# facebookresearch/holo_diffusion

Hardware: AMD Instinct MI355X
Metric: denoise-steps/sec + rendered-rays/sec, 64^3x32 grid @400^2 render (higher is better)
Workload: dtype f32

## Files before the change

### holo_diffusion_amd/csrc/holo_kernels.h

```cpp
#pragma once
#include <stddef.h>
#include <stdint.h>
#include <string.h>

#include "../../include/holo_abi.h"
#include "attn_plan.h"
#include "bwd_plan.h"
#include "conv_plan.h"
#include "conv_weights.h"
#include "holo_knobs.h"
#include "render_plan.h"

struct HoloCtx {
  int device;
  int num_cus;
  int deterministic = 0;
};

namespace holo {

int conv_launch(const ConvParams& p, void* stream);
int conv_s2_bf16_launch(const ConvParams& p, void* stream);
int conv1x1_qkv_bf16_launch(const ConvParams& p, void* stream);
int conv1x1_bf16_stream_launch(const ConvParams& p, void* stream);
int conv_wino3_launch(const ConvParams& p, void* stream);
int conv_bf16p_launch(const ConvParams& p, void* stream);
int repack_conv_weight_wino3_launch(const float* w, float* out, int Cout, int Cin, int src_taps, int CoutP, int CinP,
                                    void* stream);

int gemm_launch(const GemmParams& p, void* stream);
inline int gemm_batch_launch(const float* A, int lda, const float* B, int ldb, int b_kmajor, float* C, int ldc, int M, int N,
                             int K, int nb, int64_t sa, int64_t sb, int64_t sc, void* stream) {
  GemmParams g;
  memset(&g, 0, sizeof g);
  g.A = A, g.B = B, g.C = C;
  g.M = M, g.Nn = N, g.K = K;
  g.lda = lda, g.ldb = ldb, g.ldc = ldc;
  g.nb0 = nb, g.nb1 = 1;
  g.sa0 = sa, g.sb0 = sb, g.sc0 = sc;
  g.b_kmajor = b_kmajor;
  g.alpha = 1.f;
  return gemm_launch(g, stream);
}

int flash_attn_launch(const AttnParams& p, void* stream);
int flash_attn_bf16v2_launch(const AttnParams& p, void* work, int out_bf16, int ksplit, int lazy, void* stream, int packed = 0);

int softmax_rows_launch(float* s, int64_t rows, int cols, void* stream);

int ncdhw_to_ndhwc_launch(const float* in, float* out, int N, int C, int64_t V, int tanh_flag, void* stream,
                          int out_bf16 = 0);
int ndhwc_to_ncdhw_launch(const float* in, float* out, int N, int C, int64_t V, void* stream, int in_bf16 = 0);
int f32_to_bf16_launch(const float* in, float* out_bf16, int64_t n, void* stream);

int gn_stats_launch(const float* x, double* partial, int N, int C, int64_t V, void* stream, int x_bf16 = 0);

int gn_finalize_launch(const double* part0, int C0, int B0, const double* part1, int C1, int B1, int N, int64_t V,
                       int groups, float eps, const float* gamma, const float* beta, const float* film,
                       int film_stride, int film_cout, float* coef, void* stream, float* moments = nullptr);

int time_embed_launch(const int64_t* t, int N, int mc, int ted, const float* w1, const float* b1, const float* w2,
                      const float* b2, float* emb, float* emb_silu, int load_kind, void* stream);

int rows_linear_launch(const float* in, const float* w, const float* bias, float* out, int N, int rows, int K,
                       void* stream);

int ddpm_step_launch(const float* tables, int T, const int64_t* timesteps, int batch, int64_t per, const float* x_t,
                     const float* model_out, const float* noise, int clip, float* sample, float* pred_xstart,
                     void* stream);
int ddpm_step_philox_launch(const float* tables, int T, const int64_t* timesteps, int batch, int64_t per, const float* x_t,
                            const float* model_out, uint64_t seed, const uint32_t* row_streams, uint64_t offset, int clip,
                            float* sample, float* pred_xstart, float* noise_out, int ncdhw_channels, void* stream);
int ddim_step_launch(const float* coefs, int batch, int64_t per, const float* x_t, const float* model_out,
                     const float* noise, int clip, float* sample, float* pred_xstart, void* stream);
int ddim_step_philox_launch(const float* coefs, int batch, int64_t per, const float* x_t, const float* model_out,
                            uint64_t seed, const uint32_t* row_streams, uint64_t offset, int clip, float* sample,
                            float* pred_xstart, float* noise_out, int ncdhw_channels, void* stream);
int ddpm_step_guided_launch(const float* tables, int T, const int64_t* timesteps, const float* variances, int batch,
                            int64_t per, const float* x_t, const float* model_out, const float* grad, const float* noise,
                            int clip, float* sample, float* pred_xstart, void* stream);
int ddpm_step_guided_philox_launch(const float* tables, int T, const int64_t* timesteps, const float* variances, int batch,
                                   int64_t per, const float* x_t, const float* model_out, const float* grad, uint64_t seed,
                                   const uint32_t* row_streams, uint64_t offset, int clip, float* sample,
                                   float* pred_xstart, float* noise_out, int ncdhw_channels, void* stream);
int ddim_step_guided_launch(const float* coefs, int batch, int64_t per, const float* x_t, const float* model_out,
                            const float* grad, const float* noise, int clip, float* sample, float* pred_xstart,
                            void* stream);
int ddim_step_guided_philox_launch(const float* coefs, int batch, int64_t per, const float* x_t, const float* model_out,
                                   const float* grad, uint64_t seed, const uint32_t* row_streams, uint64_t offset, int clip,
                                   float* sample, float* pred_xstart, float* noise_out, int ncdhw_channels, void* stream);
int dpm_step_launch(const float* coefs, int batch, int64_t per, const float* x_t, const float* model_out,
                    const float* hist1, const float* hist2, int clip, float* sample, float* pred_xstart, void* stream);
int ddpm_step_inpaint_launch(const float* tables, int T, const int64_t* timesteps, const float* known_coefs, int batch,
                             int64_t per, int channels, int ncdhw, const float* x_t, const float* model_out,
                             const float* x0_known, const float* mask, const float* noise, const float* noise_known,
                             int clip, float* sample, float* pred_xstart, void* stream);
int ddpm_step_inpaint_philox_launch(const float* tables, int T, const int64_t* timesteps, const float* known_coefs, int batch,
                                    int64_t per, int channels, int ncdhw, const float* x_t, const float* model_out,
                                    const float* x0_known, const float* mask, uint64_t seed, const uint32_t* row_streams,
                                    uint64_t offset, int clip, float* sample, float* pred_xstart, float* noise_out,
                                    float* noise_known_out, void* stream);
int q_sample_launch(const float* coefs, int batch, int64_t per, const float* x, const float* noise, float* out, void* stream);
int q_sample_philox_launch(const float* coefs, int batch, int64_t per, const float* x, uint64_t seed,
                           const uint32_t* row_streams, uint64_t offset, float* out, float* noise_out, int ncdhw_channels,
                           void* stream);
int tanh_launch(const float* x, float* y, int64_t n, void* stream);
int copy_sys_launch(const float* src, float* dst, int64_t n, void* stream);
#define HIP_TRY(expr)                                                                        \
  do {                                                                                       \
    hipError_t _e = (expr);                                                                  \
    if (_e != hipSuccess) {                                                                  \
      holo::set_error("%s failed: %s (%s:%d)", #expr, hipGetErrorString(_e), __FILE__, __LINE__); \
// ... 307 lines not shown
```

### holo_diffusion_amd/csrc/holo_knobs.h

```cpp
#pragma once

#include <stdint.h>
#include <stdlib.h>

namespace holo {

#ifdef HOLO_EMU
constexpr bool EMU_BUILD = true;
#else
constexpr bool EMU_BUILD = false;
#endif

constexpr int64_t KNOB_UNSET = INT64_MIN;

#define HOLO_KNOBS(X)                                                                                                      \
  X(num_cus, "HOLO_NUM_CUS", POS, 0, CTX, "planners size grids and split-K for this many CUs (default: the device's)")     \
  X(conv_wino, "HOLO_CONV_WINO", INT, 1, HANDLE, "0: no Winograd copies of the conv weights (forward and dgrad)")          \
  X(conv_wino3, "HOLO_CONV_WINO3", INT, 1, HANDLE_PLAN, "0: no F(2x2x2, 3x3x3) copies / conv_wino3_kernel never chosen")   \
  X(keep_intermediates, "HOLO_KEEP_INTERMEDIATES", CH, '1', HANDLE,                                                        \
    "1: the plan releases no activation, holo_unet_fetch_block works")                                                     \
  X(render_v1, "HOLO_RENDER_V1", SET, 0, HANDLE, "the ray-per-column render kernel for everything")                        \
  X(render2_nw, "HOLO_RENDER2_NW", INT, 0, HANDLE, "8: the 8-wave form of render2_kernel's 12-wave configurations")        \
  X(render2_nrm_nw, "HOLO_RENDER2_NRM_NW", INT, 0, HANDLE,                                                                 \
    "8: rendered normals two waves per SIMD instead of 10 waves (the emulation build always runs 8)")                      \
  X(render_wgs, "HOLO_RENDER_WGS", POS, 0, HANDLE, "persistent render workgroups (default: one per CU)")                   \
  X(render_xcd, "HOLO_RENDER_XCD", RAW, KNOB_UNSET, HANDLE,                                                                \
    "XCD ranges of the render tile order (default 8; 2 in the emulation build; <= 1: plain order)")                        \
  X(render_tail, "HOLO_RENDER_TAIL", RAW, KNOB_UNSET, HANDLE,                                                              \
    "4-ray tiles at the end of every XCD range handed out as single rays (default: about two rounds; 3 in the "            \
    "emulation build; 0: off)")                                                                                            \
  X(render_static_tiles, "HOLO_RENDER_STATIC_TILES", SET, 0, HANDLE, "static tile stride instead of the dynamic hand-out") \
  X(render_timeline, "HOLO_RENDER_TIMELINE", SET, 0, HANDLE, "per-phase clocks of every render launch (synchronises!)")    \
  X(mlp_mean_bwd_chunk, "HOLO_MLP_MEAN_BWD_CHUNK", POS, 0, HANDLE,                                                         \
    "voxels per chunk of holo_mlp_mean_backward (default: what fits 4 GiB of rows; the emulation build: always 2048)")     \
  X(conv_wino_small, "HOLO_CONV_WINO_SMALL", INT, 1, PLAN, "0: under-filled levels take 64-voxel tiles, not Winograd")     \
  X(conv_force_tz2, "HOLO_CONV_FORCE_TZ2", INT, 0, PLAN, "1: 128-voxel tiles (hence the Winograd kernels) on small grids") \
  X(conv_qkv_fused, "HOLO_CONV_QKV_FUSED", INT, 1, PLAN, "0: row-tile qkv convolution + attn_pack_kernel")                 \
  X(conv1x1_bf16_stream, "HOLO_CONV1X1_BF16_STREAM", INT, 1, PLAN, "0: the row-tile kernel for bf16 1x1x1 convolutions")   \
  X(conv1x1_stream_min_m, "HOLO_CONV1X1_STREAM_MIN_M", INT, 131072, PLAN,                                                  \
    "rows from which a raw-input fp32 1x1x1 convolution streams (0: never)")                                               \
  X(conv1x1_small, "HOLO_CONV1X1_SMALL", INT, 1, PLAN, "0: the row-tile kernel for the fp32 attention's 1x1x1 convs")      \
  X(conv_s2t, "HOLO_CONV_S2T", INT, -1, PLAN, "stride-2 bf16 halo kernel: 0 never, 1 wherever defined (default: by fill)") \
  X(conv_bf16t, "HOLO_CONV_BF16T", INT, -1, PLAN, "bf16 wide-tile kernel: 0 never, 1 everywhere (default: by fill / K)")   \
  X(conv_bf16p, "HOLO_CONV_BF16P", INT, -1, PLAN,                                                                          \
    "its persistent form: 0 never, 1 every wide-tile launch, 2 activated input too (default: raw input)")                  \
  X(conv_bf16p_wgs, "HOLO_CONV_BF16P_WGS", INT, 0, PLAN, "at most this many persistent workgroups (0: no cap)")            \
  X(conv_wino3_min_items, "HOLO_CONV_WINO3_MIN_ITEMS", INT, KNOB_UNSET, PLAN,                                              \
    "work items from which conv_wino3_kernel runs (default: num_cus / 2)")                                                 \
  X(conv_wino3_up, "HOLO_CONV_WINO3_UP", INT, 1, PLAN,                                                                     \
    "0: upsampling convolutions on conv_wino3_kernel's generic form (64 pseudo-taps), not its 27-tap form")               \
  X(no_skip_fusion, "HOLO_NO_SKIP_FUSION", SET, 0, PLAN, "a ResBlock's 1x1x1 skip always as its own launch")               \
  X(skip_fusion_below_r, "HOLO_SKIP_FUSION_BELOW_R", RAW, 64, PLAN,                                                        \
    "exact fp32: the skip is fused into the second convolution below this grid edge")                                      \
  X(side_lane_cus, "HOLO_SIDE_LANE_CUS", INT, 128, PLAN,                                                                   \
    "exact fp32 inference: CUs the skip half of a split up-path concat convolution is planned for (0: nothing is split)")  \
  X(side_lane_min_r, "HOLO_SIDE_LANE_MIN_R", INT, 32, PLAN, "smallest grid edge whose concat convolutions are split")      \
  X(side_lane_fork_r, "HOLO_SIDE_LANE_FORK_R", INT, 8, PLAN,                                                               \
    "the side lane starts in front of the first descent level whose grid edge is at most this")                            \
  X(no_flash_attn, "HOLO_NO_FLASH_ATTN", SET, 0, PLAN, "attention as GEMM + softmax + GEMM")                               \
  X(bf16_flash_min_t, "HOLO_BF16_FLASH_MIN_T", RAW, 1024, PLAN, "tokens from which the bf16 mode takes its bf16 attention") \
  X(flash_split, "HOLO_FLASH_SPLIT", INT, 0, PLAN, "key splits of the fp32 attention, clamped to [1, T/128] (0: by fill)") \
  X(flash_v2_ksplit, "HOLO_FLASH_V2_KSPLIT", INT, 0, PLAN,                                                                 \
    "key splits of the bf16 attention: 1..8 dividing T into multiples of 128, else ignored")                               \
  X(attn_exact, "HOLO_ATTN_EXACT", SET, 0, PLAN, "bf16 attention: the exact loop alone, no LAZY pass")                     \
  X(debug_timestep_load, "HOLO_DEBUG_TIMESTEP_LOAD", INT, 0, PLAN, "how time_embed_kernel loads the timesteps (see it)")   \
  X(dgrad_s2_direct, "HOLO_DGRAD_S2_DIRECT", CH, '1', PLAN, "1: conv_dgrad_s2_kernel for every Downsample dgrad")          \
  X(wgrad_tiles, "HOLO_WGRAD_TILES", POS, 0, PLAN, "> 0: the tile weight-gradient kernel instead of the row-staged one")   \
  X(wgrad_reduce_tile_min, "HOLO_WGRAD_REDUCE_TILE_MIN", RAW, 1024, PLAN,                                                  \
    "64-element tiles from which the weight-gradient reduce runs its tile form")                                           \
  X(debug_plan, "HOLO_DEBUG_PLAN", SET, 0, PLAN, "[plan] lines on stderr: what every convolution / attention launches")    \
  X(viewpool_bwd_v1, "HOLO_VIEWPOOL_BWD_V1", CH, '1', CALL, "1: the register-accumulating view-pool backward kernel")      \
  HOLO_KNOBS_DEV(X)

#ifdef HOLO_DEV_PROBES
#define HOLO_KNOBS_DEV(X)                                                                                                  \
  X(viewpool_bwd_probe, "HOLO_VIEWPOOL_BWD_PROBE", RAW, KNOB_UNSET, CALL,                                                  \
    "view-pool backward: 0 no pass 2, 2 pass 2 without its atomics, 10 + k the atomics of map k alone")                    \
  X(viewpool_bwd_occ, "HOLO_VIEWPOOL_BWD_OCC", CH, '3', CALL, "view-pool backward: 3 = the 166-register build")
#else
#define HOLO_KNOBS_DEV(X)
#endif

typedef int64_t knob_INT_t, knob_RAW_t, knob_POS_t;
typedef bool knob_SET_t, knob_CH_t;
static inline int64_t knob_INT(const char* e, int64_t dflt) { return e && e[0] ? strtoll(e, nullptr, 10) : dflt; }
static inline int64_t knob_RAW(const char* e, int64_t dflt) { return e ? atoll(e) : dflt; }
static inline bool knob_SET(const char* e, int) { return e != nullptr; }
static inline bool knob_CH(const char* e, char c) { return e && e[0] == c; }
static inline int64_t knob_POS(const char* e, int) { return e && atoll(e) > 0 ? atoll(e) : 0; }

struct Knobs {
#define HOLO_KNOB_FIELD(field, env, kind, dflt, when, doc) knob_##kind##_t field;
  HOLO_KNOBS(HOLO_KNOB_FIELD)
#undef HOLO_KNOB_FIELD
  static Knobs from_env() {
    Knobs k;
#define HOLO_KNOB_READ(field, env, kind, dflt, when, doc) k.field = knob_##kind(getenv(env), dflt);
    HOLO_KNOBS(HOLO_KNOB_READ)
#undef HOLO_KNOB_READ
    return k;
  }
};

}
```

### holo_diffusion_amd/csrc/kernels_misc.hip

```cpp
#include <stdlib.h>

#include "holo_common.h"
#include "holo_kernels.h"

namespace holo {
namespace {

__global__ __launch_bounds__(256) void ncdhw_to_ndhwc_kernel(const float* __restrict__ in, float* __restrict__ out,
                                                             int C, int64_t V, int tanh_flag, int out_bf16) {
  __shared__ float tile[32][33];
  const int n = blockIdx.z;
  const int64_t v0 = (int64_t)blockIdx.x * 32;
  const int c0 = blockIdx.y * 32;
  const int tx = threadIdx.x & 31, ty = threadIdx.x >> 5;
  in += (int64_t)n * C * V;
  const int64_t obase = (int64_t)n * C * V;
  for (int j = ty; j < 32; j += 8) {
    const int c = c0 + j;
    const int64_t v = v0 + tx;
    float x = 0.f;
    if (c < C && v < V) x = in[(int64_t)c * V + v];
    if (tanh_flag) x = tanhf(x);
    tile[j][tx] = x;
  }
  __syncthreads();
  for (int j = ty; j < 32; j += 8) {
    const int64_t v = v0 + j;
    const int c = c0 + tx;
    if (c < C && v < V) {
      if (out_bf16)
        reinterpret_cast<uint16_t*>(out)[obase + v * C + c] = (uint16_t)(pack_bf16x2(tile[tx][j], 0.f) & 0xffffu);
      else
        out[obase + v * C + c] = tile[tx][j];
    }
  }
}

__global__ __launch_bounds__(256) void f32_to_bf16_kernel(const float4* __restrict__ in, float4* __restrict__ out, int64_t n8) {
  for (int64_t i = (int64_t)blockIdx.x * blockDim.x + threadIdx.x; i < n8; i += (int64_t)gridDim.x * blockDim.x) {
    const float4 a = in[2 * i], b = in[2 * i + 1];
    out[i] = make_float4(__uint_as_float(pack_bf16x2(a.x, a.y)), __uint_as_float(pack_bf16x2(a.z, a.w)),
                         __uint_as_float(pack_bf16x2(b.x, b.y)), __uint_as_float(pack_bf16x2(b.z, b.w)));
  }
}

__global__ __launch_bounds__(256) void ndhwc_to_ncdhw_kernel(const float* __restrict__ in, float* __restrict__ out,
                                                             int C, int64_t V, int in_bf16) {
  __shared__ float tile[32][33];
  const int n = blockIdx.z;
  const int64_t v0 = (int64_t)blockIdx.x * 32;
  const int c0 = blockIdx.y * 32;
  const int tx = threadIdx.x & 31, ty = threadIdx.x >> 5;
  const int64_t ibase = (int64_t)n * C * V;
  out += (int64_t)n * C * V;
  for (int j = ty; j < 32; j += 8) {
    const int64_t v = v0 + j;
// ... 45 lines not shown
      fs[3] += t.w;
      fq[0] += t.x * t.x;
      fq[1] += t.y * t.y;
      fq[2] += t.z * t.z;
      fq[3] += t.w * t.w;
      if (++cnt == 32) {
#pragma unroll
        for (int e = 0; e < 4; ++e) {
          ds[e] += fs[e];
          dq[e] += fq[e];
          fs[e] = 0.f;
          fq[e] = 0.f;
        }
        cnt = 0;
      }
    }
#pragma unroll
    for (int e = 0; e < 4; ++e) {
      ds[e] += fs[e];
      dq[e] += fq[e];
    }
  }
#pragma unroll
  for (int e = 0; e < 4; ++e) {
    red[tid * 8 + e] = ds[e];
    red[tid * 8 + 4 + e] = dq[e];
  }
  __syncthreads();
  if (tid < cq) {
    double s[8] = {0, 0, 0, 0, 0, 0, 0, 0};
    for (int r = 0; r < rows; ++r)
#pragma unroll
      for (int e = 0; e < 8; ++e) s[e] += red[(r * cq + tid) * 8 + e];
    double* dst = partial + (((int64_t)n * gridDim.x + blockIdx.x) * C + tid * 4) * 2;
#pragma unroll
    for (int e = 0; e < 4; ++e) {
      dst[e * 2 + 0] = s[e];
      dst[e * 2 + 1] = s[4 + e];
    }
  }
}

__device__ __forceinline__ double shfl_xor_f64(double v, int mask) {
  unsigned long long b;
  memcpy(&b, &v, 8);
  const float lo = __shfl_xor(__uint_as_float((uint32_t)(b & 0xffffffffull)), mask);
  const float hi = __shfl_xor(__uint_as_float((uint32_t)(b >> 32)), mask);
  b = (unsigned long long)__float_as_uint(lo) | ((unsigned long long)__float_as_uint(hi) << 32);
  double r;
  memcpy(&r, &b, 8);
  return r;
}

__global__ __launch_bounds__(256) void gn_finalize_kernel(const double* __restrict__ part0, int C0, int B0,
                                                          const double* __restrict__ part1, int C1, int B1, int64_t V,
                                                          int groups, float eps, const float* __restrict__ gamma,
                                                          const float* __restrict__ beta,
                                                          const float* __restrict__ film, int film_stride,
                                                          int film_cout, float* __restrict__ coef,
                                                          float* __restrict__ moments) {
  __shared__ double rs[4], rq[4];
  const int g = blockIdx.x, n = blockIdx.y, tid = threadIdx.x;
  const int Cin = C0 + C1;
  const int cpg = Cin / groups;
  float pg = 0.f, pb = 0.f, psc = 0.f, psh = 0.f;
  if (tid < cpg) {
    const int c = g * cpg + tid;
    pg = gamma[c];
    pb = beta[c];
    if (film) {
      psc = film[(int64_t)n * film_stride + c];
      psh = film[(int64_t)n * film_stride + film_cout + c];
    }
  }
  double s = 0.0, sq = 0.0;
  {
    const int c_lo = g * cpg, c_hi = c_lo + cpg;
    const int c_mid = c_lo < C0 ? (c_hi < C0 ? c_hi : C0) : c_lo;
    for (int half = 0; half < 2; ++half) {
      const int ca = half == 0 ? c_lo : c_mid, cb = half == 0 ? c_mid : c_hi;
      const int nch = cb - ca;
      if (nch <= 0) continue;
      const double* p = half == 0 && ca < C0 ? part0 : part1;
      const int Cs = p == part0 ? C0 : C1, B = p == part0 ? B0 : B1;
      const int cs0 = p == part0 ? ca : ca - C0;
      const int64_t total = (int64_t)B * nch;
      const double* base = p + ((int64_t)n * B * Cs + cs0) * 2;
      const bool pow2 = (nch & (nch - 1)) == 0;
      const int sh = 31 - __builtin_clz((unsigned)nch);
      auto rec = [&](int64_t j64) -> int64_t {
        const unsigned j = (unsigned)j64;
        const unsigned q = pow2 ? (j >> sh) : j / (unsigned)nch;
        const unsigned r = pow2 ? (j & (unsigned)(nch - 1)) : j - q * (unsigned)nch;
        return ((int64_t)q * Cs + r) * 2;
      };
      int64_t i = tid;
      for (; i + 15 * 256 < total; i += 16 * 256) {
        double2 v[16];
#pragma unroll
        for (int u = 0; u < 16; ++u) {
          const int64_t j = i + u * 256;
          v[u] = *reinterpret_cast<const double2*>(base + rec(j));
        }
#pragma unroll
        for (int u = 0; u < 16; ++u) {
          s += v[u].x;
          sq += v[u].y;
        }
      }
      for (; i + 7 * 256 < total; i += 8 * 256) {
        double2 v[8];
#pragma unroll
        for (int u = 0; u < 8; ++u) {
          const int64_t j = i + u * 256;
          v[u] = *reinterpret_cast<const double2*>(base + rec(j));
        }
#pragma unroll
        for (int u = 0; u < 8; ++u) {
          s += v[u].x;
          sq += v[u].y;
        }
      }
      for (; i < total; i += 256) {
        const double2 v = *reinterpret_cast<const double2*>(base + rec(i));
        s += v.x;
        sq += v.y;
      }
    }
  }
#pragma unroll
  for (int o = 32; o >= 1; o >>= 1) {
    s += shfl_xor_f64(s, o);
    sq += shfl_xor_f64(sq, o);
  }
  if ((tid & 63) == 0) {
    rs[tid >> 6] = s;
    rq[tid >> 6] = sq;
  }
  __syncthreads();
  if (tid < cpg) {
    const int c = g * cpg + tid;
    const double cnt = (double)cpg * (double)V;
    const double mean = (((rs[0] + rs[1]) + rs[2]) + rs[3]) / cnt;
    double var = (((rq[0] + rq[1]) + rq[2]) + rq[3]) / cnt - mean * mean;
    if (var < 0.0) var = 0.0;
    const double rstd = 1.0 / sqrt(var + (double)eps);
    double a = rstd * (double)pg;
    double b = (double)pb - mean * a;
    if (film) {
      const double sc = 1.0 + (double)psc;
      const double sh = (double)psh;
      a *= sc;
      b = b * sc + sh;
    }
    coef[((int64_t)n * Cin + c) * 2 + 0] = (float)a;
    coef[((int64_t)n * Cin + c) * 2 + 1] = (float)b;
    if (moments) {
      moments[((int64_t)n * Cin + c) * 2 + 0] = (float)mean;
      moments[((int64_t)n * Cin + c) * 2 + 1] = (float)rstd;
    }
  }
}

__global__ __launch_bounds__(256) void time_embed_kernel(const int64_t* __restrict__ t, int mc, int ted,
                                                         const float* __restrict__ w1, const float* __restrict__ b1,
                                                         const float* __restrict__ w2, const float* __restrict__ b2,
                                                         float* __restrict__ emb, float* __restrict__ emb_silu,
                                                         int load_kind) {
  __shared__ float te[256];
  __shared__ float h1[1024];
  const int n = blockIdx.x;
  const int tid = threadIdx.x;
  float tv;
  if (load_kind == 1) {
    tv = (float)t[n];
  } else if (load_kind == 2) {
    const int64_t* tp = t + n;
    HOLO_LAUNDER(tp);
    tv = (float)*tp;
  } else {
    tv = (float)holo_ld_sys(t + n);
  }
  const int half = mc / 2;
  for (int i = tid; i < mc; i += 256) {
    float v = 0.f;
    if (i < 2 * half) {
      const int k = i < half ? i : i - half;
      const float freq = expf((-9.210340371976184f * (float)k) / (float)half);
      const float arg = tv * freq;
      v = i < half ? cosf(arg) : sinf(arg);
    }
    te[i] = v;
  }
  __syncthreads();
  for (int j = tid; j < ted; j += 256) {
    float acc = 0.f;
    const float* w = w1 + (int64_t)j * mc;
    for (int k = 0; k < mc; ++k) acc = fmaf(w[k], te[k], acc);
    acc += b1[j];
    h1[j] = acc / (1.0f + expf(-acc));
  }
  __syncthreads();
  for (int j = tid; j < ted; j += 256) {
    float acc = 0.f;
    const float* w = w2 + (int64_t)j * ted;
    for (int k = 0; k < ted; ++k) acc = fmaf(w[k], h1[k], acc);
    acc += b2[j];
    emb[(int64_t)n * ted + j] = acc;
    emb_silu[(int64_t)n * ted + j] = acc / (1.0f + expf(-acc));
  }
}

__global__ __launch_bounds__(256) void rows_linear_kernel(const float* __restrict__ in, const float* __restrict__ w,
                                                          const float* __restrict__ bias, float* __restrict__ out,
// ... 568 lines not shown
    const int ci = cc * 32 + (lane >> 4) * 8 + e2 * 2;
    const float v0 = (ci < Cin && co < Cout) ? holo_ld_sys(w + ((int64_t)co * Cin + ci) * taps + tap) : 0.f;
    const float v1 = (ci + 1 < Cin && co < Cout) ? holo_ld_sys(w + ((int64_t)co * Cin + ci + 1) * taps + tap) : 0.f;
    const uint32_t h = pack_bf16x2(v0, v1);
    const float r0 = v0 - __uint_as_float(h << 16), r1 = v1 - __uint_as_float(h & 0xffff0000u);
    const uint32_t m = pack_bf16x2(r0, r1);
    const uint32_t l = pack_bf16x2(r0 - __uint_as_float(m << 16), r1 - __uint_as_float(m & 0xffff0000u));
    o32[i] = h;
    o32[total + i] = m;
    o32[2 * total + i] = l;
    {
      const int nc16 = CinP >> 4, ns32 = CoutP >> 5;
      int64_t b2 = i >> 8;
      const int sl2 = (int)(b2 % ns32);
      b2 /= ns32;
      const int cc2 = (int)(b2 % nc16);
      const int tap2 = (int)(b2 / nc16);
      const int co2 = sl2 * 32 + (lane & 31);
      const int ci2 = cc2 * 16 + (lane >> 5) * 8 + e2 * 2;
      const float u0 = (ci2 < Cin && co2 < Cout) ? w[((int64_t)co2 * Cin + ci2) * taps + tap2] : 0.f;
      const float u1 = (ci2 + 1 < Cin && co2 < Cout) ? w[((int64_t)co2 * Cin + ci2 + 1) * taps + tap2] : 0.f;
      o32[3 * total + i] = pack_bf16x2(u0, u1);
    }
  }
}

}

int ncdhw_to_ndhwc_launch(const float* in, float* out, int N, int C, int64_t V, int tanh_flag, void* stream, int out_bf16) {
  dim3 grid((unsigned)cdiv(V, 32), (unsigned)cdiv(C, 32), (unsigned)N);
  HOLO_LAUNCH(ncdhw_to_ndhwc_kernel, grid, dim3(256), stream, in, out, C, V, tanh_flag, out_bf16);
  return 0;
}
int ndhwc_to_ncdhw_launch(const float* in, float* out, int N, int C, int64_t V, void* stream, int in_bf16) {
  dim3 grid((unsigned)cdiv(V, 32), (unsigned)cdiv(C, 32), (unsigned)N);
  HOLO_LAUNCH(ndhwc_to_ncdhw_kernel, grid, dim3(256), stream, in, out, C, V, in_bf16);
  return 0;
}

int gn_stats_launch(const float* x, double* partial, int N, int C, int64_t V, void* stream, int x_bf16) {
  if ((C & 3) || (C >> 2) > 256) {
    set_error("gn_stats: unsupported C=%d", C);
    return -1;
  }
  int B, vpb;
  gn_stats_geometry(C, V, &B, &vpb);
  dim3 grid((unsigned)B, (unsigned)N);
  HOLO_LAUNCH(gn_stats_kernel, grid, dim3(256), stream, x, partial, C, V, vpb, x_bf16);
  return 0;
}

int gn_finalize_launch(const double* part0, int C0, int B0, const double* part1, int C1, int B1, int N, int64_t V,
                       int groups, float eps, const float* gamma, const float* beta, const float* film,
                       int film_stride, int film_cout, float* coef, void* stream, float* moments) {
  const int Cin = C0 + C1;
  if (Cin % groups || Cin / groups > 256) {
    set_error("gn_finalize: C=%d not compatible with %d groups", Cin, groups);
    return -1;
  }
  dim3 grid((unsigned)groups, (unsigned)N);
  HOLO_LAUNCH(gn_finalize_kernel, grid, dim3(256), stream, part0, C0, B0, part1, C1, B1, V, groups, eps, gamma, beta,
              film, film_stride, film_cout, coef, moments);
  return 0;
}

int time_embed_launch(const int64_t* t, int N, int mc, int ted, const float* w1, const float* b1, const float* w2,
                      const float* b2, float* emb, float* emb_silu, int load_kind, void* stream) {
  if (mc > 256 || ted > 1024) {
    set_error("time_embed: model_channels=%d too large", mc);
    return -1;
  }
  HOLO_LAUNCH(time_embed_kernel, dim3((unsigned)N), dim3(256), stream, t, mc, ted, w1, b1, w2, b2, emb, emb_silu, load_kind);
  return 0;
}

int rows_linear_launch(const float* in, const float* w, const float* bias, float* out, int N, int rows, int K,
                       void* stream) {
  dim3 grid((unsigned)cdiv(rows, 4), (unsigned)N);
  HOLO_LAUNCH(rows_linear_kernel, grid, dim3(256), stream, in, w, bias, out, rows, K);
  return 0;
}

static bool step_shape_ok(const char* name, int64_t per, int ncdhw_channels = 0) {
  if (per & 3) {
    set_error("%s: elems_per_sample must be a multiple of 4", name);
    return false;
  }
  if (ncdhw_channels < 0 || (ncdhw_channels & 3) || (ncdhw_channels > 0 && per % ncdhw_channels)) {
    set_error("%s: ncdhw_channels must be 0 (channels-last tensors) or a multiple of 4 that divides elems_per_sample",
              name);
    return false;
  }
  return true;
}
static dim3 step_grid(int64_t per, int batch) { return dim3((unsigned)cdiv(per / 4, 256), (unsigned)batch); }
#define HOLO_LAUNCH_PHILOX_STEP(kernel, ncdhw_channels, row_streams, ...) \
  do {                                                                    \
    if (ncdhw_channels && row_streams)                                    \
      HOLO_LAUNCH((kernel<true, true>), __VA_ARGS__);                     \
    else if (ncdhw_channels)                                              \
      HOLO_LAUNCH((kernel<true, false>), __VA_ARGS__);                    \
    else if (row_streams)                                                 \
      HOLO_LAUNCH((kernel<false, true>), __VA_ARGS__);                    \
    else                                                                  \
      HOLO_LAUNCH((kernel<false, false>), __VA_ARGS__);                   \
  } while (0)

int ddpm_step_launch(const float* tables, int T, const int64_t* timesteps, int batch, int64_t per, const float* x_t,
                     const float* model_out, const float* noise, int clip, float* sample, float* pred_xstart,
                     void* stream) {
  if (!step_shape_ok("ddpm_step", per)) return -1;
  HOLO_LAUNCH(ddpm_step_kernel, step_grid(per, batch), dim3(256), stream, tables, T, timesteps, per, x_t, model_out, noise,
              clip, sample, pred_xstart);
// ... 219 lines not shown
```

### holo_diffusion_amd/csrc/unet_exec.cpp

```cpp
#include <math.h>
#include <stdarg.h>
#include <stdio.h>
#include <stdlib.h>
#include <string.h>

#include <algorithm>
#include <map>
#include <optional>
#include <string>
#include <vector>

#include "../../include/holo_abi.h"
#include "conv_weights.h"
#include "holo_common.h"
#include "holo_kernels.h"
#include "unet_plan.h"
#include "unet_train_plan.h"

namespace holo {

static thread_local char g_err[512] = "";
void set_error(const char* fmt, ...) {
  va_list ap;
  va_start(ap, fmt);
// ... 37 lines not shown
  std::vector<void*> join_events;
};

namespace {

bool params_set(const HoloUnet* u, const char* entry) {
  for (auto& s : u->d.params)
    if (!s.set) {
      set_error("%s: parameter '%s' has not been set", entry, s.name.c_str());
      return false;
    }
  return true;
}

int ensure_train_plan(HoloUnet* u, const char* entry, int batch, void* ws, size_t ws_bytes) {
  if (!u->tplan.built_for(batch, ws)) {
    if (u->d.compute_mode != 0) {
      set_error("holo_unet_backward: the backward pass runs in the fp32 mode only");
      return HOLO_E_UNSUPPORTED;
    }
    if (!params_set(u, "holo_unet_backward")) return HOLO_E_STATE;
    TrainPlanner tp(&u->d, u->dgrad, batch, ws, u->tplan);
    tp.build();
    int rc = 0;
    if (!tp.err.empty()) {
      set_error("%s", tp.err.c_str());
      rc = HOLO_E_STATE;
    } else if (!tp.pl.regions_ok()) {
      set_error("internal: small-buffer regions overflow");
      rc = HOLO_E_INVALID;
    }
    if (rc) {
      u->tplan.invalidate();
      return rc;
    }
  }
  if (ws_bytes < u->tplan.bytes) {
    set_error("%s: workspace too small (%zu < %zu)", entry, ws_bytes, u->tplan.bytes);
    u->tplan.invalidate();
    return HOLO_E_WORKSPACE;
  }
  return 0;
}

int ensure_plan(HoloUnet* u, int batch, void* ws) {
  if (u->plan.built_for(batch, ws)) return 0;
  if (!params_set(u, "holo_unet_forward")) return HOLO_E_STATE;
  if (u->d.batch_invariant && u->d.compute_mode != 0) {
    set_error("holo_unet_forward: the batch-invariant plan is exact-fp32 only");
    return HOLO_E_UNSUPPORTED;
  }
  Planner pl(&u->d, batch, ws, u->plan);
  pl.build();
  int rc = 0;
  if (!pl.err.empty()) {
    set_error("holo_unet_forward: %s", pl.err.c_str());
    rc = HOLO_E_UNSUPPORTED;
  } else if (!pl.regions_ok()) {
    set_error("internal: small-buffer regions overflow");
    rc = HOLO_E_INVALID;
  }
  if (rc) u->plan.invalidate();
  return rc;
}

int run_op(const HoloUnet* u, const Op& op, int N, const float* x, const int64_t* t, float* y, void* stream) {
  switch (op.kind) {
    case OP_IN:
      return ncdhw_to_ndhwc_launch(x, op.in.dst, N, op.in.C, op.in.V, 0, stream, op.in.dst_bf16);
    case OP_TEMB:
      return time_embed_launch(t, N, u->d.cfg.model_channels, u->d.ted, op.temb.w1, op.temb.b1, op.temb.w2, op.temb.b2,
                               op.temb.emb, op.temb.emb_silu, op.temb.load_kind, stream);
    case OP_EMBLIN:
      return rows_linear_launch(op.emblin.emb_silu, op.emblin.w, op.emblin.b, op.emblin.out, N, u->d.emb_rows, u->d.ted, stream);
    case OP_STATS:
      return gn_stats_launch(op.stats.x, op.stats.part, N, op.stats.C, op.stats.V, stream, op.stats.x_bf16);
    case OP_FINAL: {
      const GnFinalize& f = op.fin;
      return gn_finalize_launch(f.part0, f.C0, f.B0, f.part1, f.C1, f.B1, N, f.V, f.groups, 1e-5f, f.gamma, f.beta, f.film,
                                f.film_stride, f.film_cout, f.coef, stream, f.moments);
    }
    case OP_CONV:
      return conv_launch(op.conv, stream);
    case OP_GEMM:
      return gemm_launch(op.gemm, stream);
    case OP_SOFTMAX:
      return softmax_rows_launch(op.softmax.S, op.softmax.rows, op.softmax.cols, stream);
    case OP_FLASH: {
      const Flash& f = op.flash;
      if (f.form == 2) return flash_attn_bf16v2_launch(f.attn, f.packed, f.out_bf16, f.ksplit, f.lazy, stream, f.operands_packed);
      return flash_attn_launch(f.attn, stream);
    }
    case OP_OUT:
      return ndhwc_to_ncdhw_launch(op.out.src, y, N, op.out.C, op.out.V, stream);
  }
  return 0;
}

int ensure_lanes(HoloUnet* u, int n_joins) {
#ifndef HOLO_EMU
  if (!u->side_stream) HIP_TRY(hipStreamCreateWithFlags((hipStream_t*)&u->side_stream, hipStreamNonBlocking));
  for (void** e : {&u->fork_event, &u->tail_event})
    if (!*e) HIP_TRY(hipEventCreateWithFlags((hipEvent_t*)e, hipEventDisableTiming));
  while ((int)u->join_events.size() < n_joins) {
    hipEvent_t e;
    HIP_TRY(hipEventCreateWithFlags(&e, hipEventDisableTiming));
    u->join_events.push_back(e);
  }
#endif
  (void)u, (void)n_joins;
  return 0;
}

template <class Run>
int run_lanes(HoloUnet* u, const Plan& plan, void* stream, Run run) {
  int rc = 0;
#ifdef HOLO_EMU
  for (size_t i = 0; i < plan.ops.size() && !rc; ++i) rc = run((int)i, plan.ops[i], stream);
#else
  if (!plan.n_joins) {
    for (size_t i = 0; i < plan.ops.size() && !rc; ++i) rc = run((int)i, plan.ops[i], stream);
    return rc ? (rc < 0 ? rc : HOLO_E_INVALID) : 0;
  }
  if ((rc = ensure_lanes(u, plan.n_joins))) return rc;
  const hipStream_t main = (hipStream_t)stream, side = (hipStream_t)u->side_stream;
  bool forked = false;
  hipError_t he = hipSuccess;
  for (size_t i = 0; i < plan.ops.size() && !rc && he == hipSuccess; ++i) {
    const Op& op = plan.ops[i];
    if (op.fork) {
      if ((he = hipEventRecord((hipEvent_t)u->fork_event, main)) != hipSuccess) break;
      if ((he = hipStreamWaitEvent(side, (hipEvent_t)u->fork_event, 0)) != hipSuccess) break;
      forked = true;
// ... 220 lines not shown
    return HOLO_E_INVALID;
  }
  if (s.is_conv()) {
    if (const int rc = pack_conv_weights((const float*)dev_ptr, s.w, stream)) return rc;
  } else {
    if (copy_sys_launch((const float*)dev_ptr, s.w.f32, s.numel, stream)) return HOLO_E_INVALID;
  }
  s.set = true;
  return 0;
}

int holo_unet_set_compute_dtype(HoloUnet* net, int dtype) {
  if (!net || (dtype != HOLO_DTYPE_F32 && dtype != HOLO_DTYPE_BF16 && dtype != HOLO_DTYPE_F32_BF16X3)) {
    set_error("holo_unet_set_compute_dtype: HOLO_DTYPE_F32, HOLO_DTYPE_BF16 or HOLO_DTYPE_F32_BF16X3");
    return HOLO_E_INVALID;
  }
  const int mode = dtype == HOLO_DTYPE_BF16 ? 1 : dtype == HOLO_DTYPE_F32_BF16X3 ? 2 : 0;
  if (mode != 0 && net->d.batch_invariant) {
    set_error("holo_unet_set_compute_dtype: the batch-invariant plan is exact-fp32 only; turn it off first "
              "(holo_unet_set_batch_invariant(net, 0))");
    return HOLO_E_UNSUPPORTED;
  }
  if (mode != net->d.compute_mode) {
    net->d.compute_mode = mode;
    net->plan.invalidate();
    net->ws_cache.clear();
  }
  return 0;
}

int holo_unet_set_batch_invariant(HoloUnet* net, int on) {
  if (!net) {
    set_error("holo_unet_set_batch_invariant: null net");
    return HOLO_E_INVALID;
  }
  if (on && net->d.compute_mode != 0) {
    set_error("holo_unet_set_batch_invariant: batch-invariant plans are exact-fp32 only (compute dtype HOLO_DTYPE_F32); "
              "the bf16 and bf16x3 modes are not supported");
    return HOLO_E_UNSUPPORTED;
  }
  if ((on != 0) != net->d.batch_invariant) {
    net->d.batch_invariant = on != 0;
    net->plan.invalidate();
  }
  return 0;
}

size_t holo_unet_workspace_bytes(HoloUnet* net, int batch) {
  if (!net || batch < 1) return 0;
  const std::pair<int, bool> key(batch, net->d.batch_invariant);
  auto it = net->ws_cache.find(key);
  if (it != net->ws_cache.end()) return it->second;
  Plan sizing;
  Planner(&net->d, batch, nullptr, sizing).build();
  net->ws_cache[key] = sizing.bytes;
  return sizing.bytes;
}

int holo_unet_forward(HoloUnet* net, int batch, const float* x, const int64_t* timesteps, float* y, void* workspace,
                      size_t workspace_bytes, void* stream) {
  if (!net || !x || !timesteps || !y || !workspace || batch < 1) {
    set_error("holo_unet_forward: null/invalid argument");
    return HOLO_E_INVALID;
  }
  int rc = ensure_plan(net, batch, workspace);
  if (rc) return rc;
  if (workspace_bytes < net->plan.bytes) {
    set_error("holo_unet_forward: workspace too small (%zu < %zu)", workspace_bytes, net->plan.bytes);
    return HOLO_E_WORKSPACE;
  }
  return run_plan(net, net->plan, x, timesteps, y, stream);
}

int holo_unet_forward_cl(HoloUnet* net, int batch, const float* x_cl, const int64_t* timesteps, float* y_cl, void* workspace,
                         size_t workspace_bytes, void* stream) {
  if (!net || !x_cl || !timesteps || !y_cl || !workspace || batch < 1) {
    set_error("holo_unet_forward_cl: null/invalid argument");
    return HOLO_E_INVALID;
  }
  int rc = ensure_plan(net, batch, workspace);
  if (rc) return rc;
  const Plan& plan = net->plan;
  if (workspace_bytes < plan.bytes) {
    set_error("holo_unet_forward_cl: workspace too small (%zu < %zu)", workspace_bytes, plan.bytes);
    return HOLO_E_WORKSPACE;
  }
  if (plan.cl_refusal) {
    set_error("%s", plan.cl_refusal);
    return HOLO_E_UNSUPPORTED;
  }
  const bool bf16_storage = net->d.compute_mode == 1;
  return run_lanes(net, plan, stream, [&](int i, const Op& op, void* st) {
    if (op.kind == OP_IN && bf16_storage)
      return f32_to_bf16_launch(x_cl, op.in.dst, (int64_t)batch * op.in.C * op.in.V, st) ? (int)HOLO_E_INVALID : 0;
    if (op.kind == OP_IN || op.kind == OP_OUT) return 0;
    if (i == plan.first_conv || i == plan.last_conv) {
      Op o2 = op;
      if (i == plan.first_conv && !bf16_storage) o2.conv.src0 = x_cl;
      if (i == plan.last_conv) o2.conv.out = y_cl;
      return run_op(net, o2, batch, x_cl, timesteps, y_cl, st);
    }
    return run_op(net, op, batch, x_cl, timesteps, y_cl, st);
  });
}

int holo_unet_fetch_block(HoloUnet* net, const char* tag, float* dst, int64_t dst_capacity, int64_t* numel,
                          void* workspace, void* stream) {
// ... 575 lines not shown
```

### holo_diffusion_amd/csrc/unet_plan.cpp

```cpp
#include "unet_plan.h"

#include <stdio.h>

#include <algorithm>

namespace holo {
namespace unetplan {

void build_structure(UnetDesc* u) {
  const HoloUnetCfg& c = u->cfg;
  const int mc = c.model_channels;
  int ch = c.channel_mult[0] * mc;
  char buf[128];
  u->inputs.clear();
  u->outputs.clear();
  u->middle.clear();
  u->inputs.push_back({Block{B_CONV, "input_blocks.0.0", c.in_channels, ch}});
  std::vector<int> chans{ch};
  int ds = 1, idx = 1;
  auto has_attn = [&](int d) {
    for (int i = 0; i < c.n_attention_resolutions; ++i)
      if (c.attention_resolutions[i] == d) return true;
    return false;
  };
// ... 738 lines not shown
  head.coef = coef;
  head.act = 1;
  head.out_f32 = true;
  emit_conv(head);
  y_out = y;
  release(h);
  {
    Op op = make_op(OP_OUT);
    op.out.src = ptr<float>(y.off);
    op.out.C = c.out_channels;
    op.out.V = vox(R);
    ops.push_back(op);
  }
  release(y);
  if (knobs.debug_plan) {
    int n_fin = 0, n_conv = 0, n_split = 0;
    for (const Op& o : ops) {
      n_fin += o.kind == OP_FINAL;
      if (o.kind != OP_CONV) continue;
      ++n_conv;
      n_split += o.conv.nsplit > 1;
    }
    fprintf(stderr, "[plan] batch %d: %zu ops | %d convs, %d of them split-K (+ a reduce launch) | %d gn_finalize launches\n", N, ops.size(),
            n_conv, n_split, n_fin);
  }
  find_cl_ends();
  plan.batch = N;
  plan.ws = ptr<void>(0);
  plan.bytes = arena_base + arena.peak;
}
void Planner::find_cl_ends() {
  const float* in_buf = nullptr;
  const float* out_buf = nullptr;
  int first = -1, last = -1;
  for (size_t i = 0; i < ops.size(); ++i) {
    const Op& op = ops[i];
    if (op.kind == OP_IN) in_buf = op.in.dst;
    if (op.kind == OP_OUT) out_buf = op.out.src;
    if (op.kind == OP_CONV) {
      if (first < 0 && in_buf) first = (int)i;
      last = (int)i;
    }
  }
  plan.first_conv = first;
  plan.last_conv = last;
  if (first < 0 || !in_buf || !out_buf || ops[first].conv.src0 != in_buf || ops[first].conv.src1 ||
      ops[last].conv.out != out_buf || first == last) {
    plan.cl_refusal = "holo_unet_forward_cl: this plan's first / last convolution cannot take the caller's tensors";
  } else if (bfs() && (ops[last].conv.out_bf16 || !ops[first].conv.in_bf16)) {
    plan.cl_refusal = "holo_unet_forward_cl: unexpected storage types at the ends of the bf16 plan";
  }
}

}
}
```

### holo_diffusion_amd/csrc/unet_plan.h

```cpp
#pragma once
#include <math.h>
#include <stddef.h>
#include <stdint.h>
#include <string.h>

#include <map>
#include <optional>
#include <string>
#include <utility>
#include <vector>

#include "../../include/holo_abi.h"
#include "attn_plan.h"
#include "bwd_plan.h"
#include "conv_plan.h"
#include "conv_weights.h"
#include "holo_knobs.h"

namespace holo {
namespace unetplan {

enum BlockKind { B_CONV, B_RES, B_ATTN, B_DOWN, B_UP, B_HEAD };
struct Block {
  BlockKind kind;
// ... 55 lines not shown
      fl.erase(fl.begin() + i);
    }
    if (!fl.empty() && fl.back().first + fl.back().second == top) {
      top = fl.back().first;
      fl.pop_back();
    }
  }
};

struct Act {
  size_t off = 0, bytes = 0;
  size_t stats_off = 0, stats_bytes = 0;
  int stats_B = 0;
  int C = 0, R = 0;
  int refs = 0;
};

struct Tape {
  Block b;
  Act x0, x1, h1, out;
  bool has_x1 = false;
  size_t coefA = 0, coefB = 0, momA = 0, momB = 0;
  const float* film = nullptr;
  size_t qkv = 0, a = 0;
  bool has_skip = false;
};

enum OpKind { OP_IN = 1, OP_TEMB, OP_EMBLIN, OP_STATS, OP_FINAL, OP_CONV, OP_GEMM, OP_SOFTMAX, OP_FLASH, OP_OUT };
struct LayoutIn { float* dst; int C; int64_t V; int dst_bf16; };
struct LayoutOut { const float* src; int C; int64_t V; };
struct TimeEmbed {
  const float *w1, *b1, *w2, *b2;
  float *emb, *emb_silu;
  int load_kind;
};
struct EmbLinears {
  const float *emb_silu, *w, *b;
  float* out;
};
struct GnStats {
  const float* x;
  double* part;
  int C, x_bf16;
  int64_t V;
};
struct GnFinalize {
  const double *part0, *part1;
  int C0, B0, C1, B1;
  int64_t V;
  const float *gamma, *beta, *film;
  int film_stride, film_cout;
  float *coef, *moments;
  int groups;
};
struct Softmax { float* S; int64_t rows; int cols; };
struct Flash {
  AttnParams attn;
  int form;
  float* packed;
  int out_bf16;
  int operands_packed;
  int ksplit, lazy;
};
struct Op {
  OpKind kind;
  union {
    LayoutIn in;
    TimeEmbed temb;
    EmbLinears emblin;
    GnStats stats;
    GnFinalize fin;
    ConvParams conv;
    GemmParams gemm;
    Softmax softmax;
    Flash flash;
    LayoutOut out;
  };
  unsigned char side, fork;
  short join;
};
inline Op make_op(OpKind kind) {
  Op op;
  memset(&op, 0, sizeof op);
  op.kind = kind;
  op.join = -1;
  return op;
}

struct Plan {
  int batch = -1;
  void* ws = nullptr;
  bool sizing = false;
  std::vector<Op> ops;
  size_t bytes = 0;
  std::map<std::string, Act> block_outputs;
  int first_conv = -1, last_conv = -1;
  const char* cl_refusal = nullptr;
  int n_joins = 0;
  bool built_for(int b, const void* w) const { return !sizing && batch == b && ws == w && !ops.empty(); }
  void invalidate() { *this = Plan(); }
};

enum BwdOpKind {
  BOP_CONV = 1, BOP_WGRAD, BOP_COLSUM, BOP_GN_BWD, BOP_ADD, BOP_SPLIT_CAT, BOP_SUMPOOL2, BOP_ZERO_INSERT2, BOP_DGRAD_S2, BOP_GEMM,
  BOP_SOFTMAX, BOP_ATTN_DS, BOP_TRANSPOSE, BOP_FILM_BWD, BOP_TEMB_BWD
};
// ... 154 lines not shown
  Act x_in, y_out;
  struct SideRange {
    size_t off, bytes;
    int join;
  };
  std::vector<SideRange> side_live;
  struct SidePart {
    Act P;
    int id = 0, join = -1;
    bool consumed = false;
  };
  std::map<std::string, SidePart> side_parts;

  Planner(const UnetDesc* u_, int N_, void* ws, Plan& plan_);
  void build();
  bool regions_ok() const { return small_top <= small_cap; }

  template <class T>
  T* ptr(size_t off) const {
    return reinterpret_cast<T*>(base + off);
  }
  int64_t vox(int R) const { return (int64_t)R * R * R; }
  bool bfs() const { return u->compute_mode == 1; }
  int plan_n() const { return u->batch_invariant && !tape ? 1 : N; }

  Act new_act(int C, int R, bool f32 = false);
  void alloc_stats(Act& a, int slabs);
  void release(Act& a);
  size_t small_alloc(size_t bytes);
  size_t scratch_alloc(size_t bytes) { return guarded(arena_base + arena.alloc(bytes), bytes); }
  void scratch_free(size_t off, size_t bytes) { arena.free(off - arena_base, bytes); }
  size_t guarded(size_t off, size_t bytes);

  void emit_stats(Act& a);
  size_t emit_finalize(const Act& x0, const Act* x1, const std::string& norm, const float* film = nullptr, int film_cout = 0);
  size_t emit_finalize_half(const Act& x, int c_first, int cpg, const std::string& norm);
  Tape& record(const Block& b, const Act& x0, const Act& out);
  ConvDesc conv_of(const std::string& layer, const Act& x, const Act& out);
  void hand_over(const ConvWeights& cw, ConvParams& p, bool skip, int cin0 = -1);
  size_t plan_conv(const ConvDesc& d, ConvParams& p);
  ConvParams place_conv(const ConvDesc& d, int* stats_slabs = nullptr);
  void emit_conv(const ConvDesc& d);

  bool side_stream_used() const { return true; }
  bool split_eligible(const Block& b, const Act& x1, int n_for);
  void plan_side_lane(const std::vector<Act>& hs);

  Act resblock(const Block& b, Act& x0, Act* x1);
  Act attention(const Block& b, Act& x);
  Act run_layers(const std::vector<Block>& layers, Act h, Act* skip, bool release_h);
  void find_cl_ends();
};

}
}
```

Measured before the change: 174.4.

## Pre-activate GroupNorm+SiLU in finalize for deepest-level row-tile convolutions

Adds a finalize variant that, after computing the GroupNorm coefficients, writes the normalized and SiLU-activated tensor into scratch placed behind the plan. A plan pass then redirects qualifying fp32 row-tile convolutions (tiny grids of at most 64 voxels, with high tap×Cout-tile redundancy) to read this pre-activated input instead of re-applying norm+SiLU per tap and per Cout tile. It removes redundant per-tap activation arithmetic in exchange for an extra scratch buffer and an extra write/read pass on the tiny deepest-level tensors.

```diff
diff --git a/holo_diffusion_amd/csrc/holo_kernels.h b/holo_diffusion_amd/csrc/holo_kernels.h
--- a/holo_diffusion_amd/csrc/holo_kernels.h
+++ b/holo_diffusion_amd/csrc/holo_kernels.h
@@ -57,7 +57,8 @@
 
 int gn_finalize_launch(const double* part0, int C0, int B0, const double* part1, int C1, int B1, int N, int64_t V,
                        int groups, float eps, const float* gamma, const float* beta, const float* film,
-                       int film_stride, int film_cout, float* coef, void* stream, float* moments = nullptr);
+                       int film_stride, int film_cout, float* coef, void* stream, float* moments = nullptr,
+                       const float* x0 = nullptr, const float* x1 = nullptr, float* act = nullptr, int act_silu = 0);
 
 int time_embed_launch(const int64_t* t, int N, int mc, int ted, const float* w1, const float* b1, const float* w2,
                       const float* b2, float* emb, float* emb_silu, int load_kind, void* stream);
diff --git a/holo_diffusion_amd/csrc/holo_knobs.h b/holo_diffusion_amd/csrc/holo_knobs.h
--- a/holo_diffusion_amd/csrc/holo_knobs.h
+++ b/holo_diffusion_amd/csrc/holo_knobs.h
@@ -57,6 +57,8 @@
   X(side_lane_min_r, "HOLO_SIDE_LANE_MIN_R", INT, 32, PLAN, "smallest grid edge whose concat convolutions are split")      \
   X(side_lane_fork_r, "HOLO_SIDE_LANE_FORK_R", INT, 8, PLAN,                                                               \
     "the side lane starts in front of the first descent level whose grid edge is at most this")                            \
+  X(rowtile_preact, "HOLO_ROWTILE_PREACT", INT, 1, PLAN,                                                                   \
+    "0: row-tile convolutions of the deepest level apply GroupNorm + SiLU themselves, per tap and Cout tile")              \
   X(no_flash_attn, "HOLO_NO_FLASH_ATTN", SET, 0, PLAN, "attention as GEMM + softmax + GEMM")                               \
   X(bf16_flash_min_t, "HOLO_BF16_FLASH_MIN_T", RAW, 1024, PLAN, "tokens from which the bf16 mode takes its bf16 attention") \
   X(flash_split, "HOLO_FLASH_SPLIT", INT, 0, PLAN, "key splits of the fp32 attention, clamped to [1, T/128] (0: by fill)") \
diff --git a/holo_diffusion_amd/csrc/kernels_misc.hip b/holo_diffusion_amd/csrc/kernels_misc.hip
--- a/holo_diffusion_amd/csrc/kernels_misc.hip
+++ b/holo_diffusion_amd/csrc/kernels_misc.hip
@@ -2,6 +2,7 @@
 
 #include "holo_common.h"
 #include "holo_kernels.h"
+#include "rowtile_silu.h"
 
 namespace holo {
 namespace {
@@ -153,17 +154,45 @@
   return r;
 }
 
-__global__ __launch_bounds__(256) void gn_finalize_kernel(const double* __restrict__ part0, int C0, int B0,
-                                                          const double* __restrict__ part1, int C1, int B1, int64_t V,
-                                                          int groups, float eps, const float* __restrict__ gamma,
-                                                          const float* __restrict__ beta,
-                                                          const float* __restrict__ film, int film_stride,
-                                                          int film_cout, float* __restrict__ coef,
-                                                          float* __restrict__ moments) {
-  __shared__ double rs[4], rq[4];
+struct GnPreact {
+  const float *x0, *x1;
+  float* act;
+  int silu;
+};
+constexpr int GN_PRE_TOP = 2;
+
+template <bool PRE>
+__device__ __forceinline__ void gn_finalize_body(double* rs, double* rq, float* s_ab, const double* __restrict__ part0, int C0,
+                                                 int B0, const double* __restrict__ part1, int C1, int B1, int64_t V,
+                                                 int groups, float eps, const float* __restrict__ gamma,
+                                                 const float* __restrict__ beta, const float* __restrict__ film,
+                                                 int film_stride, int film_cout, float* __restrict__ coef,
+                                                 float* __restrict__ moments, const GnPreact& pre) {
   const int g = blockIdx.x, n = blockIdx.y, tid = threadIdx.x;
   const int Cin = C0 + C1;
   const int cpg = Cin / groups;
+  const unsigned qpg = (unsigned)cpg >> 2, items = PRE ? (unsigned)V * qpg : 0u;
+  auto item_at = [&](unsigned i, int64_t& row, int& c) {
+    const unsigned v = i / qpg;
+    c = g * cpg + 4 * (int)(i - v * qpg);
+    row = (int64_t)n * V + v;
+  };
+  auto item_src = [&](int64_t row, int c) { return c < C0 ? pre.x0 + row * C0 + c : pre.x1 + row * C1 + (c - C0); };
+  float4 xr[GN_PRE_TOP];
+  const bool x_at_top = PRE && items <= (unsigned)GN_PRE_TOP * 256u;
+  if (PRE && x_at_top) {
+#pragma unroll
+    for (int u = 0; u < GN_PRE_TOP; ++u) {
+      const unsigned i = (unsigned)tid + (unsigned)u * 256u;
+      xr[u] = make_float4(0.f, 0.f, 0.f, 0.f);
+      if (i < items) {
+        int64_t row;
+        int c;
+        item_at(i, row, c);
+        xr[u] = *reinterpret_cast<const float4*>(item_src(row, c));
+      }
+    }
+  }
   float pg = 0.f, pb = 0.f, psc = 0.f, psh = 0.f;
   if (tid < cpg) {
     const int c = g * cpg + tid;
@@ -260,7 +289,63 @@
       moments[((int64_t)n * Cin + c) * 2 + 0] = (float)mean;
       moments[((int64_t)n * Cin + c) * 2 + 1] = (float)rstd;
     }
-  }
+    if (PRE) {
+      s_ab[tid * 2 + 0] = (float)a;
+      s_ab[tid * 2 + 1] = (float)b;
+    }
+  }
+  if (PRE) {
+    __syncthreads();
+    auto apply = [&](unsigned i, float4 x) {
+      int64_t row;
+      int c;
+      item_at(i, row, c);
+      const float4* ab = reinterpret_cast<const float4*>(s_ab + (c - g * cpg) * 2);
+      const float4 c01 = ab[0], c23 = ab[1];
+      float4 y = make_float4(__builtin_fmaf(x.x, c01.x, c01.y), __builtin_fmaf(x.y, c01.z, c01.w),
+                             __builtin_fmaf(x.z, c23.x, c23.y), __builtin_fmaf(x.w, c23.z, c23.w));
+      if (pre.silu) y = make_float4(silu_f(y.x), silu_f(y.y), silu_f(y.z), silu_f(y.w));
+      *reinterpret_cast<float4*>(pre.act + row * Cin + c) = y;
+    };
+    if (x_at_top) {
+#pragma unroll
+      for (int u = 0; u < GN_PRE_TOP; ++u) {
+        const unsigned i = (unsigned)tid + (unsigned)u * 256u;
+        if (i < items) apply(i, xr[u]);
+      }
+    } else {
+      for (unsigned i = (unsigned)tid; i < items; i += 256u) {
+        int64_t row;
+        int c;
+        item_at(i, row, c);
+        apply(i, *reinterpret_cast<const float4*>(item_src(row, c)));
+      }
+    }
+  }
+}
+
+__global__ __launch_bounds__(256) void gn_finalize_kernel(const double* __restrict__ part0, int C0, int B0,
+                                                          const double* __restrict__ part1, int C1, int B1, int64_t V,
+                                                          int groups, float eps, const float* __restrict__ gamma,
+                                                          const float* __restrict__ beta,
+                                                          const float* __restrict__ film, int film_stride,
+                                                          int film_cout, float* __restrict__ coef,
+                                                          float* __restrict__ moments) {
+  __shared__ double rs[4], rq[4];
+  gn_finalize_body<false>(rs, rq, nullptr, part0, C0, B0, part1, C1, B1, V, groups, eps, gamma, beta, film, film_stride,
+                          film_cout, coef, moments, GnPreact{nullptr, nullptr, nullptr, 0});
+}
+__global__ __launch_bounds__(256) void gn_finalize_act_kernel(const double* __restrict__ part0, int C0, int B0,
+                                                              const double* __restrict__ part1, int C1, int B1, int64_t V,
+                                                              int groups, float eps, const float* __restrict__ gamma,
+                                                              const float* __restrict__ beta,
+                                                              const float* __restrict__ film, int film_stride,
+                                                              int film_cout, float* __restrict__ coef,
+                                                              float* __restrict__ moments, GnPreact pre) {
+  __shared__ double rs[4], rq[4];
+  __shared__ __attribute__((aligned(16))) float s_ab[512];
+  gn_finalize_body<true>(rs, rq, s_ab, part0, C0, B0, part1, C1, B1, V, groups, eps, gamma, beta, film, film_stride, film_cout,
+                         coef, moments, pre);
 }
 
 __global__ __launch_bounds__(256) void time_embed_kernel(const int64_t* __restrict__ t, int mc, int ted,
@@ -935,13 +1020,29 @@
 
 int gn_finalize_launch(const double* part0, int C0, int B0, const double* part1, int C1, int B1, int N, int64_t V,
                        int groups, float eps, const float* gamma, const float* beta, const float* film,
-                       int film_stride, int film_cout, float* coef, void* stream, float* moments) {
+                       int film_stride, int film_cout, float* coef, void* stream, float* moments, const float* x0,
+                       const float* x1, float* act, int act_silu) {
   const int Cin = C0 + C1;
   if (Cin % groups || Cin / groups > 256) {
     set_error("gn_finalize: C=%d not compatible with %d groups", Cin, groups);
     return -1;
   }
+  const int cpg = Cin / groups;
+  if ((int64_t)(B0 > B1 ? B0 : B1) * cpg >= ((int64_t)1 << 31)) {
+    set_error("gn_finalize: %d slabs of %d channels per group: more than 2^31 records per run", B0 > B1 ? B0 : B1, cpg);
+    return -1;
+  }
   dim3 grid((unsigned)groups, (unsigned)N);
+  if (act) {
+    if ((cpg & 3) || (C0 & 3) || !x0 || (C1 > 0 && !x1) || V * (cpg >> 2) >= ((int64_t)1 << 31)) {
+      set_error("gn_finalize: the activated tensor needs whole 4-channel quads per group and source (%d + %d channels, %d groups) "
+                "and fewer than 2^31 of them per group (%lld voxels)", C0, C1, groups, (long long)V);
+      return -1;
+    }
+    HOLO_LAUNCH(gn_finalize_act_kernel, grid, dim3(256), stream, part0, C0, B0, part1, C1, B1, V, groups, eps, gamma, beta,
+                film, film_stride, film_cout, coef, moments, GnPreact{x0, x1, act, act_silu});
+    return 0;
+  }
   HOLO_LAUNCH(gn_finalize_kernel, grid, dim3(256), stream, part0, C0, B0, part1, C1, B1, V, groups, eps, gamma, beta,
               film, film_stride, film_cout, coef, moments);
   return 0;
diff --git a/holo_diffusion_amd/csrc/unet_exec.cpp b/holo_diffusion_amd/csrc/unet_exec.cpp
--- a/holo_diffusion_amd/csrc/unet_exec.cpp
+++ b/holo_diffusion_amd/csrc/unet_exec.cpp
@@ -113,6 +113,7 @@
   }
   Planner pl(&u->d, batch, ws, u->plan);
   pl.build();
+  if (pl.err.empty()) preactivate_rowtile(u->plan, pl.knobs);
   int rc = 0;
   if (!pl.err.empty()) {
     set_error("holo_unet_forward: %s", pl.err.c_str());
@@ -139,7 +140,7 @@
     case OP_FINAL: {
       const GnFinalize& f = op.fin;
       return gn_finalize_launch(f.part0, f.C0, f.B0, f.part1, f.C1, f.B1, N, f.V, f.groups, 1e-5f, f.gamma, f.beta, f.film,
-                                f.film_stride, f.film_cout, f.coef, stream, f.moments);
+                                f.film_stride, f.film_cout, f.coef, stream, f.moments, f.x0, f.x1, f.act, f.act_silu);
     }
     case OP_CONV:
       return conv_launch(op.conv, stream);
@@ -466,7 +467,9 @@
   auto it = net->ws_cache.find(key);
   if (it != net->ws_cache.end()) return it->second;
   Plan sizing;
-  Planner(&net->d, batch, nullptr, sizing).build();
+  Planner pl(&net->d, batch, nullptr, sizing);
+  pl.build();
+  preactivate_rowtile(sizing, pl.knobs);
   net->ws_cache[key] = sizing.bytes;
   return sizing.bytes;
 }
diff --git a/holo_diffusion_amd/csrc/unet_plan.cpp b/holo_diffusion_amd/csrc/unet_plan.cpp
--- a/holo_diffusion_amd/csrc/unet_plan.cpp
+++ b/holo_diffusion_amd/csrc/unet_plan.cpp
@@ -814,5 +814,53 @@
   }
 }
 
-}
-}
+
+const char* preact_refusal(const PreactShape& s) {
+  if (s.cpg % 4 != 0) return "a group is no whole number of 4-channel quads";
+  if (s.C0 % 4 != 0) return "a quad would straddle the seam of the concat";
+  if (s.V > PREACT_MAX_VOX) return "the tensor is too large for the finalize launch";
+  if (s.redundancy < PREACT_MIN_REDUNDANCY) return "the convolution repeats too little of the activation";
+  return nullptr;
+}
+
+Preact preactivate_rowtile(Plan& plan, const Knobs& knobs) {
+  Preact r;
+  std::vector<Op>& ops = plan.ops;
+  const int N = plan.batch;
+  const uintptr_t base = reinterpret_cast<uintptr_t>(plan.ws);
+  r.scratch_off = Arena::al(plan.bytes);
+  float* const scratch = reinterpret_cast<float*>(base + r.scratch_off);
+  for (size_t i = 0; knobs.rowtile_preact && i < ops.size(); ++i) {
+    if (ops[i].kind != OP_FINAL || ops[i].side || ops[i].fin.act) continue;
+    GnFinalize& f = ops[i].fin;
+    int readers = 0;
+    for (const Op& o : ops) readers += o.kind == OP_CONV && o.conv.coef == f.coef;
+    size_t j = i + 1;
+    while (j < ops.size() && (ops[j].side || ops[j].kind != OP_CONV)) ++j;
+    if (readers != 1 || j == ops.size() || ops[j].conv.coef != f.coef) continue;
+    ConvParams& p = ops[j].conv;
+    const int Cin = p.C0 + p.C1;
+    const int64_t V = (int64_t)p.ID * p.IH * p.IW;
+    if (p.kernel != ConvKernel::RowTile || p.bf16 != 0 || p.in_bf16 != 0 || p.ups || p.N != N || f.moments) continue;
+    if (Cin != f.C0 + f.C1 || V != f.V || f.groups < 1 || Cin % f.groups) continue;
+    const PreactShape shape{Cin / f.groups, p.C0, V, p.ksz * p.ksz * p.ksz * ((p.Cout + 63) / 64)};
+    if (preact_refusal(shape)) continue;
+    ConvParams q = p;
+    q.src0 = scratch, q.C0 = Cin, q.src1 = nullptr, q.C1 = 0, q.coef = nullptr;
+    if (!conv_can_launch(q)) continue;
+    f.x0 = p.src0, f.x1 = p.src1, f.act = scratch, f.act_silu = p.act;
+    q.act = 0;
+    p = q;
+    const size_t bytes = (size_t)N * (size_t)V * Cin * sizeof(float);
+    if (bytes > r.scratch_bytes) r.scratch_bytes = bytes;
+    ++r.pairs;
+  }
+  if (r.pairs) plan.bytes = r.scratch_off + Arena::al(r.scratch_bytes);
+  if (knobs.debug_plan)
+    fprintf(stderr, "[plan] batch %d: %d finalize + row-tile convolution pairs pre-activated (%zu bytes of scratch behind the plan)\n",
+            N, r.pairs, r.pairs ? Arena::al(r.scratch_bytes) : (size_t)0);
+  return r;
+}
+
+}
+}
diff --git a/holo_diffusion_amd/csrc/unet_plan.h b/holo_diffusion_amd/csrc/unet_plan.h
--- a/holo_diffusion_amd/csrc/unet_plan.h
+++ b/holo_diffusion_amd/csrc/unet_plan.h
@@ -131,6 +131,9 @@
   int film_stride, film_cout;
   float *coef, *moments;
   int groups;
+  const float *x0, *x1;
+  float* act;
+  int act_silu;
 };
 struct Softmax { float* S; int64_t rows; int cols; };
 struct Flash {
@@ -391,5 +394,19 @@
   void find_cl_ends();
 };
 
-}
-}
+struct PreactShape {
+  int cpg, C0;
+  int64_t V;
+  int redundancy;
+};
+constexpr int64_t PREACT_MAX_VOX = 64;
+constexpr int PREACT_MIN_REDUNDANCY = 16;
+const char* preact_refusal(const PreactShape& s);
+struct Preact {
+  int pairs = 0;
+  size_t scratch_off = 0, scratch_bytes = 0;
+};
+Preact preactivate_rowtile(Plan& plan, const Knobs& knobs);
+
+}
+}
```

Measured after the change: 178.0, median of 6. +2.1%, better.
